# lxm0851/mp3

Hardware: AMD Instinct MI355X
Metric: stereo MP3 frames/s (128 kbps 44.1 kHz) at 1/2/4/8 GPU; % HBM roofline (higher is better)
Workload: dtype f32; 1 GPU; C3: full Layer III decode (Huffman->PCM), 65536 streams x 32 frames per GPU per step; streams_per_gpu=65536, hz=44100, seed=default, parallelism=streams sharded, 1 process per GPU, no data-path collective

## Files before the change

### abx/variants.py

```python
#!/usr/bin/env python3
import sys

import stage

KERNELS = ["mp3d_demux.hip", "mp3d_huffman.hip", "mp3d_synth.hip", "mp3d_demux_dev.h", "mp3d_huffman_dev.h", "mp3d_internal.h"]


def variant(name, reps):
    srcs = {k: open("mp3_amd/csrc/" + k).read() for k in KERNELS}
    flags = [b for a, b in reps if a == "FLAGS"]
    reps = [(a, b) for a, b in reps if a != "FLAGS"]
    for a, b in reps:
        assert any(a in s for s in srcs.values()), (name, a)
        srcs = {k: s.replace(a, b) for k, s in srcs.items()}
    stage.build("/tmp/vars/" + name, "build_ab/%s.so" % name, srcs, extra=flags)


W4H = ("__global__ void __launch_bounds__(HUFF_BLOCK) k_huffman(",
       "__global__ void __launch_bounds__(HUFF_BLOCK) __attribute__((amdgpu_waves_per_eu(4, 8))) k_huffman(")
_QS = "            /* ---------------- phase Q: requantise + stereo -> LDS ---------- */"
_IS = "            /* ---------------- phase I: alias + IMDCT + overlap ------------ */"
_MS = "            /* ---------------- phase M: matrixing on the matrix cores ------- */"
_WS = "            /* ---------------- phase W: 512-tap window -> PCM --------------- */"

# ... 713 lines not shown
                                   "+v"(xbp[6]), "+v"(xbp[7]));"""),
]

VARS["PHT"] = [
    ("    float *const sBuf = Wd.buf;\n",
     "    float *const sBuf = Wd.buf;\n    unsigned long long ph_[4] = {0ull, 0ull, 0ull, 0ull}, tQ_ = 0ull, tI_ = 0ull, tM_ = 0ull, tW_ = 0ull;\n"),
    (_QS, "            tQ_ = clock64();\n" + _QS),
    (_IS, "            tI_ = clock64(); ph_[0] += tI_ - tQ_;\n" + _IS),
    (_MS, "            tM_ = clock64(); ph_[1] += tM_ - tI_;\n" + _MS),
    (_WS, "            tW_ = clock64(); ph_[2] += tW_ - tM_;\n" + _WS),
    ("            wave_sync(); /* X reads done before the next granule's xr */",
     "            wave_sync(); /* X reads done before the next granule's xr */\n            ph_[3] += clock64() - tW_;"),
    ("    if (f1 == F && PF != 1) {",
     "    if ((blockIdx.x == 0 || blockIdx.x == 4000) && threadIdx.x == 0 && !SRC_XR && !LSF)\n"
     "        printf(\"PHT blk %d Q %llu I %llu M %llu W %llu\\n\", (int)blockIdx.x, ph_[0], ph_[1], ph_[2], ph_[3]);\n"
     "    if (f1 == F && PF != 1) {"),
]

VARS["PHT2"] = [
    ("    float *const sBuf = Wd.buf;\n",
     "    float *const sBuf = Wd.buf;\n    unsigned long long ph_[8] = {0ull, 0ull, 0ull, 0ull, 0ull, 0ull, 0ull, 0ull}, tQ_ = 0ull, tI_ = 0ull, tM_ = 0ull, tW_ = 0ull, tE_ = 0ull, t1_ = 0ull, t2_ = 0ull;\n"),
    (_QS, "            tQ_ = clock64(); if (tE_) ph_[7] += tQ_ - tE_;\n" + _QS),
    ("                (void)m12a;\n", "                (void)m12a;\n                t1_ = clock64(); ph_[4] += t1_ - tQ_;\n"),
    ("                xin();\n                } /* !fusedq */", "                t2_ = clock64(); ph_[5] += t2_ - t1_;\n                xin();\n                } /* !fusedq */"),
    (_IS, "            tI_ = clock64(); ph_[0] += tI_ - tQ_; ph_[6] += tI_ - t2_;\n" + _IS),
    (_MS, "            tM_ = clock64(); ph_[1] += tM_ - tI_;\n" + _MS),
    (_WS, "            tW_ = clock64(); ph_[2] += tW_ - tM_;\n" + _WS),
    ("            wave_sync(); /* X reads done before the next granule's xr */",
     "            wave_sync(); /* X reads done before the next granule's xr */\n            tE_ = clock64(); ph_[3] += tE_ - tW_;"),
    ("    if (f1 == F && PF != 1) {",
     "    if ((blockIdx.x == 0 || blockIdx.x == 4000) && threadIdx.x == 0 && !SRC_XR && !LSF)\n"
     "        printf(\"PHT2 blk %d Q %llu (Q1 %llu Q2 %llu Q3 %llu) I %llu M %llu W %llu G %llu\\n\", (int)blockIdx.x, ph_[0], ph_[4], ph_[5], ph_[6], ph_[1], ph_[2], ph_[3], ph_[7]);\n"
     "    if (f1 == F && PF != 1) {"),
]

VARS["PHT3"] = [
    ("    float *const sBuf = Wd.buf;\n",
     "    float *const sBuf = Wd.buf;\n    unsigned long long ph_[8] = {0ull, 0ull, 0ull, 0ull, 0ull, 0ull, 0ull, 0ull}, tQ_ = 0ull, t1_ = 0ull, ta_ = 0ull, tb_ = 0ull, tc_ = 0ull;\n"),
    ("                (void)m12a;\n", "                (void)m12a;\n                t1_ = clock64();\n"),
    ("                else read_cis(std::integral_constant<int, 5>{});\n",
     "                else read_cis(std::integral_constant<int, 5>{});\n                __asm__ volatile(\"s_waitcnt lgkmcnt(0)\" : \"+v\"(cis[0][0]), \"+v\"(cis[1][0]), \"+v\"(cis[0][1]), \"+v\"(cis[1][1]));\n                ta_ = clock64(); ph_[0] += ta_ - t1_;\n"),
    ("                else requant(std::integral_constant<int, 5>{});\n",
     "                else requant(std::integral_constant<int, 5>{});\n                __asm__ volatile(\"s_waitcnt lgkmcnt(0)\" : \"+v\"(xp[0][0]), \"+v\"(xp[1][0]));\n                tb_ = clock64(); ph_[1] += tb_ - ta_;\n"),
    ("                if (ms_fold) {\n",
     "                tc_ = clock64(); ph_[2] += tc_ - tb_;\n                if (ms_fold) {\n"),
    ("                xin();\n                } /* !fusedq */", "                ph_[3] += clock64() - tc_;\n                xin();\n                } /* !fusedq */"),
    ("    if (f1 == F && PF != 1) {",
     "    if ((blockIdx.x == 0 || blockIdx.x == 4000) && threadIdx.x == 0 && !SRC_XR && !LSF)\n"
     "        printf(\"PHT3 blk %d cis %llu requant %llu esc+stereo %llu scatter %llu\\n\", (int)blockIdx.x, ph_[0], ph_[1], ph_[2], ph_[3]);\n"
     "    if (f1 == F && PF != 1) {"),
]

VARS["MSZ"] = [
    ("""                            scatter(i, 0, xp[0][i] + xp[1][i]);
                            scatter(i, 1, xp[0][i] - xp[1][i]);""",
     """                            if (i < 2 || i < nlive) {
                                scatter(i, 0, xp[0][i] + xp[1][i]);
                                scatter(i, 1, xp[0][i] - xp[1][i]);
                            } else {
                                scatter(i, 0, (f32x2){0.f, 0.f});
                                scatter(i, 1, (f32x2){0.f, 0.f});
                            }"""),
]

VARS["MH"] = [
    ("    for (int f = fw; f < f1; f++) {\n        int nch, sr, mode = 0, mext = 0;",
     "    const int mlane_ = (int)(threadIdx.x & 63);\n"
     "    const uint32_t m_off_a = (uint32_t)(((mlane_ & 15) * SROW + 4 * (mlane_ >> 4)) * 4);\n"
     "    const uint32_t m_off_c = (uint32_t)((((mlane_ & 15) < 4 ? 32 + (mlane_ & 15) : 35) * SROW + 4 * (mlane_ >> 4)) * 4);\n"
# ... 329 lines not shown
```

### mp3_amd/csrc/mp3d_batch.cpp

```cpp
#include "mp3d_host.h"

using namespace mp3d;

hipError_t mp3d::state_clear(StreamState *st, int n, hipStream_t s) {
    hipError_t e = hipMemsetAsync(st, 0, sizeof(StreamState) * (size_t)n, s);
    if (e == hipSuccess)
        e = hipMemset2DAsync(&st[0].fmt, sizeof(StreamState), MP3D_STATE_FMT_BYTE, sizeof(uint32_t), (size_t)n, s);
    return e;
}

static bool poison_env() {
    const char *e = getenv("MP3D_DEBUG_POISON");
    return e && e[0] && strcmp(e, "0") != 0;
}

static int seg_frames(int n, int F, int n_cu, int min_len) {
    int seg_len = F;
    const long long want = 4LL * 4 * n_cu;
    if ((long long)n < want && F >= 2 * min_len) {
        const int nseg = (int)std::min<long long>((want + n - 1) / n, F / min_len);
        seg_len = (F + nseg - 1) / nseg;
    }
    const char *e = getenv("MP3D_SEG_FRAMES");
    if (e && atoi(e) > 0) seg_len = std::min(F, atoi(e));
// ... 167 lines not shown
    return MP3D_OK;
}

extern "C" int mp3d_batch_kernel_times(mp3d_batch *b, float *us3) {
    if (!b || !us3) return MP3D_E_ARG;
    if (!b->timing) return MP3D_E_ARG;
    HIPCHK(hipEventSynchronize(b->ev[3]));
    for (int i = 0; i < 3; i++) {
        float ms = 0;
        HIPCHK(hipEventElapsedTime(&ms, b->ev[i], b->ev[i + 1]));
        us3[i] = ms * 1000.f;
    }
    return MP3D_OK;
}

#define MP3D_WIDE_STREAMS 256
static bool demux_wide(int n) {
    const char *e = getenv("MP3D_DEMUX");
    if (e && !strcmp(e, "lane")) return true;
    if (e && !strcmp(e, "wave")) return false;
    return n >= MP3D_WIDE_STREAMS;
}

#define MP3D_WAVE_HUFF_UNITS 1024
static bool huffman_wave(int n_units) {
    const char *e = getenv("MP3D_HUFF");
    if (e && !strcmp(e, "wave")) return true;
    if (e && !strcmp(e, "lane")) return false;
    return n_units <= MP3D_WAVE_HUFF_UNITS;
}

#define MP3D_GEO_CACHE_STREAMS (1 << 30)

int mp3d::prepare_geometry(mp3d_batch *b, const uint64_t *offsets, const uint32_t *sizes, int n, hipStream_t s) {
    {
        mp3d_batch::Geo &g = b->geo[b->geo_i];
        if (n <= MP3D_GEO_CACHE_STREAMS && g.n == n && !memcmp(g.h, offsets, sizeof(uint64_t) * n) &&
            !memcmp(g.h + 2 * (size_t)n, sizes, sizeof(uint32_t) * n)) {
            HIPCHK(hipStreamWaitEvent(s, g.staged, 0));
            return MP3D_OK;
        }
    }
    b->geo_i ^= 1;
    mp3d_batch::Geo &g = b->geo[b->geo_i];
    g.n = -1;
    HIPCHK(hipEventSynchronize(g.staged));
// ... 87 lines not shown
    const bool inf_host = infos && !mapped && !is_device_ptr(infos, b->device);
    mp3d_frame_info *dinf = infos && !inf_host ? infos : b->d_infos.p;
    int r = fp ? run_front_fp(b, *fp, F, s, dinf) : run_front(b, frames, offsets, sizes, n, F, s, &sync_needed, mapped, dinf);
    if (r) return r;
    if (async && !mapped) return MP3D_E_ARG;
    const size_t PB = f32 ? sizeof(float) : sizeof(int16_t), row = 2304 * PB;
    const size_t pcm_bytes = (size_t)n * F * row;
    void *dpcm = pcm;
    const PtrKind pk = mapped ? PTR_DEV : ptr_kind(pcm, b->device);
    bool pcm_host = pk == PTR_HOST;
    if (pk != PTR_DEV) {
        r = b->d_pcm.grow(b, pcm_bytes);
        if (r) return r;
        dpcm = b->d_pcm;
        if (pk == PTR_OTHER_DEV) HIPCHK(hipMemcpyAsync(dpcm, pcm, pcm_bytes, hipMemcpyDefault, s));
    }
    DeviceCtx &dc = g_dev[b->device];
    const int seg_len = seg_len_req > 0 ? std::min(F, seg_len_req) : seg_frames(n, F, dc.n_cu, 4);
    TailPlan tp;
    r = tail_plan(b, n, F, seg_len, s, &tp);
    if (r) return r;
    if (b->poison) launch_lds_poison(dc.n_cu, s);
    launch_synth(b->rec, b->is_buf, b->meta, dc.tables, b->st, dpcm, f32, n, F, kinds, seg_len, tp.out, tp.in,
                 b->fam_ok ? b->d_work + 1 : nullptr, b->call_seq, dc.n_cu, s);
    if (b->timing) HIPCHK(hipEventRecord(b->ev[3], s));
    HIPCHK(hipGetLastError());
    tail_commit(b, n, F, seg_len, tp);
    const size_t ib = sizeof(mp3d_frame_info) * (size_t)n * F;
    if (pcm_host && !overwrite) {
        std::vector<mp3d_frame_info> tmp;
        mp3d_frame_info *hi = inf_host ? infos : nullptr;
        if (!hi) {
            tmp.resize((size_t)n * F);
            hi = tmp.data();
        }
        HIPCHK(hipMemcpyAsync(hi, dinf, ib, hipMemcpyDefault, s));
        HIPCHK(hipStreamSynchronize(s));
        std::vector<size_t> at;
        std::vector<uint8_t> kept;
        for (size_t i = 0; i < (size_t)n * F; i++) {
            const size_t w = (size_t)hi[i].samples * (size_t)hi[i].channels * PB;
            if (w >= row) continue;
            at.push_back(i);
            kept.insert(kept.end(), (const uint8_t *)pcm + i * row + w, (const uint8_t *)pcm + (i + 1) * row);
        }
        HIPCHK(hipMemcpyAsync(pcm, dpcm, pcm_bytes, hipMemcpyDeviceToHost, s));
        HIPCHK(hipStreamSynchronize(s));
// ... 245 lines not shown
```

### mp3_amd/csrc/mp3d_launch.h

```cpp
#ifndef MP3D_LAUNCH_H
#define MP3D_LAUNCH_H

#include <hip/hip_runtime.h>
#include <stdint.h>

struct StreamState; struct FrameRec; struct UnitMeta; struct DevTables;
struct RsState; struct RsCfg; struct RsPlan; struct RsLong;
struct FtState; struct FtPlan; struct FtTab;
struct LdState; struct LdPlan; struct LdTab;
struct TpState; struct TpPlan;

namespace mp3d {

hipError_t upload_demux_constants(const uint16_t *frame_bytes);
void launch_demux(const uint8_t *in, const uint64_t *in_off, const uint32_t *in_len, uint8_t *md,
                  const uint64_t *md_off, StreamState *st, FrameRec *rec, uint64_t *sideu, void *infos, int n_streams,
                  int F, int opts, bool wide, uint32_t *fam, uint32_t seq, hipStream_t strm);
void launch_demux_fp(const uint8_t *in, uint32_t len, const uint32_t *fo, uint8_t *md, StreamState *st,
                     const float *tail_in, StreamState *snap, FrameRec *rec, uint64_t *sideu, void *infos, int F,
                     int opts, hipStream_t strm);

void launch_huffman(const uint8_t *md, const uint64_t *md_off, const FrameRec *rec, const uint64_t *sideu,
                    const DevTables *tab, int16_t *is_buf, UnitMeta *meta, int n_streams, int F, int n_cu, bool wave,
                    uint32_t *work, uint32_t *rank, hipStream_t strm);

hipError_t upload_synth_constants(const float *win36, const float *is_ratio, const float *pow2q, const float *is_lsf);
hipError_t upload_frame_constants(const uint16_t *frame_bytes);
void launch_frame(const uint8_t *in_host, uint32_t in_have, const uint64_t *in_off, const uint32_t *in_len,
                  uint8_t *md, const uint64_t *md_off, StreamState *st, FrameRec *rec, uint64_t *sideu, void *infos,
                  int opts, const DevTables *tab, int16_t *is_buf, UnitMeta *meta, void *pcm, bool f32, bool lsf,
                  uint32_t *done, uint32_t seq, hipStream_t strm);
void launch_synth(const FrameRec *rec, const int16_t *is_buf, const UnitMeta *meta, const DevTables *tab,
                  StreamState *st, void *pcm, bool f32, int n_streams, int F, int kinds, int seg_len, float *st_tail,
                  const float *st_tail_in, const uint32_t *fam, uint32_t seq, int n_cu, hipStream_t strm);
void launch_synth_xr(const float *xr, const uint8_t *bt, const uint8_t *mixed, const DevTables *tab, StreamState *st,
                     int16_t *pcm, int n_streams, int F, int nch, int sr, int seg_len, float *st_tail,
                     const float *st_tail_in, hipStream_t strm);
void launch_lds_poison(int n_cu, hipStream_t strm);
void launch_gather_frames(const void *src, void *dst, const void *isrc, void *idst, const int *a, int L, int F, int k0,
                          int n_out, int bytes_per_row, hipStream_t strm);
#ifdef MP3D_WG_LDS_POISON
int wglds_probe_words();
void launch_wglds_probe(int n_cu, int n_groups, uint32_t *out, hipStream_t strm);
#endif

void launch_resample(const float *rows, const void *infos, RsState *st, const StreamState *sst, const RsCfg *cfg,
                     int out_ch, const float *tab, RsPlan *plan, int32_t *prefix, void *out, bool f32,
                     int32_t *out_count, int n, int F, long long stride, int tiles, int flush, int gapless,
                     hipStream_t strm);
void launch_resample_long(const float *rows, const void *infos, const int *a, const uint32_t *tag, const RsCfg *cfg,
                          int out_ch, const float *tab, RsLong *st, int32_t *prefix, void *out, bool f32, long long cap,
                          int L, int F, int k0, int n_out, int tiles, int first, int last, int gapless, hipStream_t strm);

void launch_features(const float *samples, const int32_t *counts, FtState *st, FtPlan *plan, const FtTab *tab, float *feat,
                     int32_t *feat_count, int n, long long sample_stride, long long feat_stride, int tiles, int flush,
                     hipStream_t strm);

// ... 19 lines not shown
```

### mp3_amd/csrc/mp3d_synth.hip

```cpp
#include "mp3d_device.h"
#include "mp3d_consts.h"
#define MP3D_DEMUX_TU frame_tu
#include "mp3d_demux_dev.h"
#include "mp3d_huffman_dev.h"
#include "mp3d_launch.h"

namespace mp3d {

__constant__ float c_win36[4][36];
__constant__ float c_is_ratio[7][2];
__constant__ float c_pow2q[4];
__constant__ float c_is_lsf[2][16][2];

__device__ __forceinline__ void dct3_9(const float *a, float *v) {
    const float C10 = 9.848077530e-01f;
    const float C20 = 9.396926208e-01f;
    const float C30 = 8.660254038e-01f;
    const float C40 = 7.660444431e-01f;
    const float C50 = 6.427876097e-01f;
    const float C70 = 3.420201433e-01f;
    const float C80 = 1.736481777e-01f;
    const float ev0 = fmaf(a[8], C80, fmaf(a[6], 0.5f, fmaf(a[4], C40, fmaf(a[2], C20, a[0]))));
    const float od0 = fmaf(a[7], C70, fmaf(a[5], C50, fmaf(a[3], C30, a[1] * C10)));
    v[0] = ev0 + od0;
// ... 163 lines not shown
    for (int i = tid; i < 32 * 16; i += NT)
        ((float *)&T.dwp[0][0])[((i & 15) >> 1) * 64 + (i >> 4) * 2 + (i & 1)] = (&tab->dwin[0][0])[i] * (F32 ? 1.0f : 32768.0f);
    if (tid < 7 + 9) {
        const float c9[7] = DCT9_KC, k9[9] = IMDCT36_K;
        T.kc[tid] = tid < 7 ? (f32x2){c9[tid], c9[tid]} : (f32x2){k9[tid - 7], -k9[tid - 7]};
    }
    if (tid < 4) T.p2q[tid] = pow2_quarter(tid);
    if (tid < 128) {
        const int l = tid & 63, c = l >> 5, j = l & 31;
        const int w = (tid >> 6) ? tab->win_b[j] : tab->win_a[j];
        T.xcol[tid >> 6][l] = (uint16_t)(18 * c * XROW + (w & 1) * 16 + (w >> 1));
    }
    for (int k = tid; k < 2 * 4 * 9; k += NT) {
        const int par = k / 36, bt = (k / 9) % 4, i = k % 9;
        const float *w = c_win36[bt];
        const float sa = (par && (i & 1)) ? -1.f : 1.f, sb = (par && !(i & 1)) ? -1.f : 1.f;
        T.wp[par][bt][i] = (f32x4){sa * w[i], sb * w[17 - i], sa * w[18 + i], sb * w[35 - i]};
    }
    if (LSF) {
        if (tid < 64) (&T.isr[0][0])[tid] = (&c_is_lsf[0][0][0])[tid];
    } else if (tid < 14) (&T.isr[0][0])[tid] = (&c_is_ratio[0][0])[tid];
}

template <bool SRC_XR, bool F32, bool LSF, int PF = 0>
__device__ __forceinline__ void synth_stream(const FrameRec *__restrict__ rec, const int16_t *__restrict__ is_buf,
                                             const UnitMeta *__restrict__ meta, const float *__restrict__ xr_in,
                                             const uint8_t *__restrict__ xr_bt, const uint8_t *__restrict__ xr_mixed,
                                             const DevTables *__restrict__ tab, StreamState *__restrict__ st,
                                             void *__restrict__ pcm, int F, int xr_nch, int xr_sr, int seg_len,
                                             float *__restrict__ st_tail, const float *__restrict__ st_tail_in,
                                             SynShared<LSF> &T, SynWave &Wd, int s, int seg, int nseg,
                                             float *xch = nullptr, uint32_t *isq = nullptr) {
    static_assert(PF == 0 || (!SRC_XR && !LSF), "PF: k_frame's MPEG-1 decode path only");
    const int f0 = seg * seg_len, f1 = min(F, f0 + seg_len);
    int fw = seg ? f0 - 1 : 0;
    int wlast = -1;
    bool from_state = seg == 0, ch1_state = false;
    if (!SRC_XR && seg > 0) {
        const uint32_t *rw = (const uint32_t *)(rec + (size_t)s * F);
        auto audio = [&](int f) {
            const uint32_t r4 = __builtin_amdgcn_readfirstlane(rw[8 * f + 4]);
            const uint32_t r6 = __builtin_amdgcn_readfirstlane(rw[8 * f + 6]);
            return (r4 & 0xFFFFu) != 0u && !(((r6 >> 8) & 0xFFu) & (REC_TAG | REC_DROP));
        };
        auto stereo = [&](int f) { return (__builtin_amdgcn_readfirstlane(rw[8 * f + 5]) >> 24) == 2u; };
        const int need = LSF ? 2 : 1;
        int found = 0, fa = f0;
// ... 218 lines not shown
            const uint32_t r5 = (uint32_t)__builtin_amdgcn_readlane((int)wr[0], 37);
            const uint32_t r6 = (uint32_t)__builtin_amdgcn_readlane((int)wr[0], 38);
            const uint32_t first_gr = (r6 >> 8) & 0xFFu;
            if (!(r4 & 0xFFFFu) || (first_gr & (REC_TAG | REC_DROP))) {
                if (f + 1 < f1) prefetch_full(2 * (f + 1));
                WAIT_VMCNT0();
                continue;
            }
            nch = (int)(r5 >> 24);
            sr = (int)((r6 >> 16) & 15u) - (LSF ? 3 : 0);
            mode = (int)(r5 >> 22) & 3;
            mext = (int)(r5 >> 20) & 3;
        }
        const uint64_t amask = nch == 2 ? ~0ull : 0xFFFFFFFFull;
        const uint32_t(*lpair)[288] = T.lpair[sr];
#pragma unroll
        for (int gr = PF == 2 ? 1 : 0; gr < (LSF || PF == 1 ? 1 : 2); gr++) {
            const int cs = PAR ? gr : 0;
            const int lane = opaque((int)(threadIdx.x & 63));
            const int ch = lane >> 5, sb = lane & 31;
            int bt0, mx0, bt1 = 0, mx1 = 0;
            if (!SRC_XR) __builtin_amdgcn_s_setprio(1);
            bool fusedq = false;
            float xf[18], up[8], dn[8];
            auto xin = [&]() {
                wave_sync();
                typedef __attribute__((address_space(3))) const f32x2 lds_cf2;
                lds_cf2 *const P = (lds_cf2 *)(uintptr_t)((uint32_t)(uintptr_t)(lds_cf32 *)(const float *)sBuf + xin_off);
#pragma unroll
                for (int i = 0; i < 9; i++) {
                    const f32x2 v = P[4 + i];
                    xf[2 * i] = v.x;
                    xf[2 * i + 1] = v.y;
                }
#pragma unroll
                for (int i = 0; i < 4; i++) {
                    const f32x2 p = P[i];
                    const f32x2 n = P[13 + i];
                    up[7 - 2 * i] = p.x;
                    up[6 - 2 * i] = p.y;
                    dn[2 * i] = n.x;
                    dn[2 * i + 1] = n.y;
                }
            };
            if (SRC_XR) {
                (void)fr;
                f32x2 cx[2][5];
#pragma unroll
                for (int c = 0; c < 2; c++)
#pragma unroll
                    for (int i = 0; i < 5; i++)
// ... 8 lines not shown
                    bt1 = __builtin_amdgcn_readlane((int)nbt, 1);
                    mx1 = bt1 == 2 ? __builtin_amdgcn_readlane((int)nbt, 3) : 0;
                }
                if (f + 1 < f1 || gr == 0) load_xr(2 * f + gr + 1);
                const int xv[2] = {bt0 == 2 ? (mx0 ? 2 : 1) : 0, bt1 == 2 ? (mx1 ? 2 : 1) : 0};
#pragma unroll
                for (int i = 0; i < 5; i++) {
                    if (i < 4 || lane < 32) {
                        const int k = lane + 64 * i;
#pragma unroll
                        for (int c = 0; c < 2; c++) {
                            if (c < nch) {
                                if (xv[c] == 0) {
                                    *(f32x2 *)&sBuf[576 * c + 2 * k] = cx[c][i];
                                } else {
                                    const uint32_t tv2 = lpair[xv[c]][k];
                                    sBuf[576 * c + ((tv2 >> 8) & 1023u)] = cx[c][i][0];
                                    sBuf[576 * c + ((tv2 >> 18) & 1023u)] = cx[c][i][1];
                                }
                            }
                        }
                    }
                }
                xin();
            } else {
                const int nzq0 = __builtin_amdgcn_readlane((int)wm[cs], 12) & 0xFFFF;
                const int nzq1 = nch == 2 ? __builtin_amdgcn_readlane((int)wm[cs], MW + 12) & 0xFFFF : 0;
                const int nzmax = nzq0 > nzq1 ? nzq0 : nzq1;
                const int nlive = nzmax <= 256 ? 2 : (nzmax <= 384 ? 3 : 5);
                uint32_t cis[2][5];
                auto read_cis = [&](auto nic) {
                    constexpr int NI = decltype(nic)::value;
#pragma unroll
                    for (int c = 0; c < 2; c++)
#pragma unroll
                        for (int i = 0; i < 5; i++)
                            cis[c][i] = i < NI ? (PAR ? isq[320 * c + 64 * i + lane] : nis[c][i]) : 0u;
                };
                if (lane < nch * MW) ((uint32_t *)&Wd.m[0])[lane] = wm[cs];
                const uint32_t m10a = (uint32_t)__builtin_amdgcn_readlane((int)wm[cs], 10);
                const uint32_t m11a = (uint32_t)__builtin_amdgcn_readlane((int)wm[cs], 11);
                const uint32_t m12a = (uint32_t)__builtin_amdgcn_readlane((int)wm[cs], 12);
                const uint32_t m10b = (uint32_t)__builtin_amdgcn_readlane((int)wm[cs], MW + 10);
                const uint32_t m11b = (uint32_t)__builtin_amdgcn_readlane((int)wm[cs], MW + 11);
                const uint32_t m12b = (uint32_t)__builtin_amdgcn_readlane((int)wm[cs], MW + 12);
                bt0 = (int)(m10a >> 8) & 0xFF;
                mx0 = (int)(m10a >> 16) & 0xFF;
                if (nch == 2) {
                    bt1 = (int)(m10b >> 8) & 0xFF;
                    mx1 = (int)(m10b >> 16) & 0xFF;
                }
                const int var[2] = {bt0 == 2 ? (mx0 ? 2 : 1) : 0, bt1 == 2 ? (mx1 ? 2 : 1) : 0};
                const bool is_on = mode == 1 && nch == 2 && (mext & 1);
                const bool ms_fold = mode == 1 && nch == 2 && mext == 2;
                fusedq = PAR && var[0] == 0 && var[1] == 0 && !is_on && !ms_fold;
                const float rsq2 = 0.70710678118654752f;
                const float msf = __int_as_float(__builtin_amdgcn_readfirstlane(ms_fold ? 0x3f3504f3 : 0x3f800000));
                auto p2q = [&](int q) { return ldexpf(T.p2q[q & 3], q >> 2) * msf; };
                if (var[0] == 0 && (nch == 1 || var[1] == 0)) {
                    const int c = lane >> 5, bl = lane & 31, j = bl < 22 ? bl : 21;
                    const uint32_t g10 = c ? m10b : m10a, g11 = c ? m11b : m11a;
                    const int gain = (int)(g10 & 0xFFu) - 210, shift = (int)(g10 >> 24) + 1;
                    const uint32_t wd = (uint32_t)__shfl((int)wm[cs], c * MW + (j >> 2));
                    const int sf = (int)(wd >> (8 * (j & 3))) & 0xFF;
                    const int pre = (g11 & 0xFFu) ? (int)(MP3D_PRETAB_BITS >> (2 * j)) & 3 : 0;
                    const float v = p2q(gain - ((sf + pre) << shift));
                    if (bl < 22) Wd.scale[c][bl] = v;
                } else {
                    const bool lng = lane < 22;
                    const int b = (lane - 22) / 3, w = lane - 22 - 3 * b;
                    auto band_scale = [&](uint32_t g10, uint32_t g11, int cbase) {
                        const int gain = (int)(g10 & 0xFFu) - 210, shift = (int)(g10 >> 24) + 1;
                        const bool mixed = ((g10 >> 16) & 0xFFu) != 0u, preflag = (g11 & 0xFFu) != 0u;
                        int j = mixed ? 8 + 3 * (b - 3) + w : 3 * b + w;
                        j = lng ? lane : (j < 0 ? 0 : (j > 39 ? 39 : j));
                        const uint32_t wd = (uint32_t)__shfl((int)wm[cs], cbase + (j >> 2));
                        const int sf = (int)(wd >> (8 * (j & 3))) & 0xFF;
                        const int pre = preflag ? (int)(MP3D_PRETAB_BITS >> (2 * (lane & 31))) & 3 : 0;
// ... 31 lines not shown
                        xf[2 * m] = *(const float *)(p43b + (t & 0x7FCu)) * sc;
                        xf[2 * m + 1] = *(const float *)(p43b + ((t >> 16) & 0x7FCu)) * sc;
                    }
                    if (__ballot((bigf & 0xF800F800u) != 0u)) {
#pragma unroll
                        for (int m = 0; m < 9; m++) {
                            const uint32_t w = iw[m];
#pragma unroll
                            for (int e = 0; e < 2; e++) {
                                const int v = (int)(int16_t)(e ? (w >> 16) : (w & 0xFFFFu));
                                const int a = v < 0 ? -v : v;
                                if ((uint32_t)(v + 256) >= 512u) {
                                    const float mag = pow43_big(a) * *(lds_cf32 *)(uintptr_t)(scb | (lpw[m] & 0xFCu));
                                    xf[2 * m + e] = v < 0 ? -mag : mag;
                                }
                            }
                        }
                    }
#pragma unroll
                    for (int k = 0; k < 8; k++) {
                        up[k] = __int_as_float(__builtin_amdgcn_update_dpp(0, __float_as_int(xf[17 - k]), 0x138, 0xF, 0xF, false));
                        dn[k] = __int_as_float(__builtin_amdgcn_update_dpp(0, __float_as_int(xf[k]), 0x130, 0xF, 0xF, false));
                    }
                } else {
                if (nlive == 2) read_cis(std::integral_constant<int, 2>{});
                else if (nlive == 3) read_cis(std::integral_constant<int, 3>{});
                else read_cis(std::integral_constant<int, 5>{});
                auto requant = [&](auto nic) {
                constexpr int NI = decltype(nic)::value;
#pragma unroll
                for (int i = 0; i < 5; i++) {
                    const bool ok = i < 4 || lane < 32;
#pragma unroll
                    for (int c = 0; c < 2; c++) {
                        if (i >= NI) {
                            XV(c, 2 * i) = 0.f;
                            XV(c, 2 * i + 1) = 0.f;
                            continue;
                        }
                        const uint32_t tv2 = ok ? lpair[var[c]][lane + 64 * i] : 0u;
                        uint32_t t;
                        __asm__("v_pk_mad_u16 %0, %1, 4, %2 op_sel_hi:[1,0,0]" : "=v"(t) : "v"(cis[c][i]), "s"(k1024));
                        bigacc |= t;
                        const float sc = *(lds_cf32 *)(uintptr_t)(sc_base[c] | (tv2 & 0xFCu));
                        XV(c, 2 * i) = *(const float *)(p43b + (t & 0x7FCu)) * sc;
                        XV(c, 2 * i + 1) = *(const float *)(p43b + ((t >> 16) & 0x7FCu)) * sc;
// ... 79 lines not shown
                        *(f32x2 *)&sBuf[576 * c + 2 * lane + 128 * i] = v;
                    } else {
                        const uint32_t tv2 = lpair[var[c]][lane + 64 * i];
                        sBuf[576 * c + ((tv2 >> 8) & 1023u)] = v.x;
                        sBuf[576 * c + ((tv2 >> 18) & 1023u)] = v.y;
                    }
                };
                if (ms_fold) {
#pragma unroll
                    for (int i = 0; i < 5; i++)
                        if (i < 4 || lane < 32) {
                            scatter(i, 0, xp[0][i] + xp[1][i]);
                            scatter(i, 1, xp[0][i] - xp[1][i]);
                        }
                } else {
#pragma unroll
                    for (int i = 0; i < 5; i++)
                        if (i < 4 || lane < 32) {
#pragma unroll
                            for (int c = 0; c < 2; c++)
                                if (c < nch) scatter(i, c, xp[c][i]);
                        }
                }
                xin();
                }
                if (PF == 0 && (LSF ? f + 1 < f1 : (gr == 0 || f + 1 < f1))) prefetch(LSF ? 2 * f + 2 : 2 * f + gr + 1, cs);
            }
            wave_sync();
#undef XV
            if (!SRC_XR) __builtin_amdgcn_s_setprio(0);
            if (PF == 2) {
                __syncthreads();
#pragma unroll
                for (int i = 0; i < 9; i++) ovp[i] = (f32x2){xch[2 * i * 64 + lane], xch[(2 * i + 1) * 64 + lane]};
            }
            const int bt = ch ? bt1 : bt0, mixed = ch ? mx1 : mx0;
            float o18[18];
            f32x2 nvp[9];
            {
                const int base = ch * 576 + 18 * sb;
                float(&x)[18] = xf;
                (void)base;
                const bool upper = (bt != 2 && sb >= 1) || (bt == 2 && mixed && sb == 1);
                const bool lower = (bt != 2 && sb <= 30) || (bt == 2 && mixed && sb == 0);
#pragma unroll
                for (int k = 0; k < 8; k++) {
                    const float lo = x[17 - k], hi = x[k];
                    const float nh = fmaf(up[k], MP3D_K_ALIAS_CA[k], hi * MP3D_K_ALIAS_CS[k]);
                    const float nl = fmaf(-dn[k], MP3D_K_ALIAS_CA[k], lo * MP3D_K_ALIAS_CS[k]);
                    x[k] = upper ? nh : hi;
                    x[17 - k] = lower ? nl : lo;
                }
                const bool long_imdct = bt != 2 || (mixed && sb < 2);
                if (long_imdct) {
                    const f32x4 *wq = T.wp[sb & 1][bt == 2 ? 0 : bt];
                    f32x2 W[9];
                    imdct36_wp(x, W, (const f32x2 *)(uintptr_t)(uint32_t)opaque((int)(uintptr_t)(lds_cf32 *)(const float *)&T.kc[0]));
#pragma unroll
                    for (int i = 0; i < 9; i++) {
                        const f32x4 q = wq[i];
                        const f32x2 o = pfma(bc(W[8 - i].y), (f32x2){q.x, q.y}, ovp[i]);
                        o18[i] = o.x;
                        o18[17 - i] = o.y;
                        nvp[i] = bc(W[8 - i].x) * (f32x2){q.z, q.w};
                    }
                } else {
                    const float sgo = (sb & 1) ? -1.f : 1.f;
                    const f32x2 sgp[2] = {(f32x2){1.f, sgo}, (f32x2){sgo, 1.f}};
                    float z[24];
#pragma unroll
                    for (int i = 0; i < 24; i++) z[i] = 0.f;
#pragma unroll
                    for (int w = 0; w < 3; w++) {
                        float h[6];
// ... 236 lines not shown
        const f32x2 sgp[2] = {(f32x2){1.f, sgo}, (f32x2){sgo, 1.f}};
        float *ovo = st_tail ? st_tail + (size_t)s * TAIL : &S.overlap[0][0][0];
        float *ffo = ovo + sizeof(S.overlap) / 4;
#pragma unroll
        for (int i = 0; i < 9; i++) {
            const f32x2 t = ovp[i] * sgp[i & 1];
            ovo[(ch * 32 + sb) * 18 + i] = t.x;
            ovo[(ch * 32 + sb) * 18 + 17 - i] = t.y;
        }
        const float hsc = F32 ? 1.0f : 1.0f / 32768.0f;
#pragma unroll
        for (int tp = 0; tp < 8; tp++) {
            ffo[(ch * MP3D_FIFO_SLOTS + 2 * tp) * 32 + sb] = hp[tp].x * hsc;
            if (2 * tp + 1 < MP3D_FIFO_SLOTS) ffo[(ch * MP3D_FIFO_SLOTS + 2 * tp + 1) * 32 + sb] = hp[tp].y * hsc;
        }
    }
}

template <bool SRC_XR, bool LSF> struct SynCfg {
    static constexpr bool DMA = !LSF;
    static constexpr int WAVES = DMA ? 8 : 4;
};

template <bool SRC_XR, bool F32, bool LSF>
__global__ void __launch_bounds__((64 * SynCfg<SRC_XR, LSF>::WAVES))
    __attribute__((amdgpu_waves_per_eu(SynCfg<SRC_XR, LSF>::DMA ? 4 : 3, 8)))
k_synth(const FrameRec *__restrict__ rec, const int16_t *__restrict__ is_buf, const UnitMeta *__restrict__ meta,
        const float *__restrict__ xr_in, const uint8_t *__restrict__ xr_bt, const uint8_t *__restrict__ xr_mixed,
        const DevTables *__restrict__ tab, StreamState *__restrict__ st, void *__restrict__ pcm, int n_streams,
        int F, int xr_nch, int xr_sr, int seg_len, float *__restrict__ st_tail,
        const float *__restrict__ st_tail_in, const uint32_t *__restrict__ fam, uint32_t seq) {
    constexpr int SYN_WAVES = SynCfg<SRC_XR, LSF>::WAVES;
    struct Lds {
        float pad_[64];
        SynWave Wv[SYN_WAVES];
        SynShared<LSF> T;
        uint32_t isq[SynCfg<SRC_XR, LSF>::DMA ? SYN_WAVES : 1][2 * 320];
    };
    static_assert(offsetof(Lds, T) + sizeof(SynShared<LSF>) <= 65536, "k_synth: tables within DS offset reach");
    static_assert(LSF || SRC_XR || sizeof(Lds) <= 160 * 1024 / 2, "k_synth: LDS for two workgroups per CU");
    __shared__ __attribute__((aligned(16))) Lds L;
    MP3D_LDS_ENTRY();
    SynShared<LSF> &T = L.T;
    SynWave *Wv = L.Wv;
    auto &s_isq = L.isq;
    if (LSF && !SRC_XR && fam && *fam != seq) return;
    if (!SRC_XR && !(LSF && fam)) {
        bool any = false;
        const int nsg = (F + seg_len - 1) / seg_len;
#pragma unroll
        for (int k = 0; k < SYN_WAVES; k++) {
            const int sk = (blockIdx.x * SYN_WAVES + k) / nsg;
            if (sk < n_streams) any |= (st[sk].kind == 2) == LSF;
        }
        if (!any) return;
    }
    synth_tables<F32, LSF, 64 * SYN_WAVES>(T, tab, threadIdx.x);
    __syncthreads();
    const int wid = __builtin_amdgcn_readfirstlane((int)(threadIdx.x >> 6));
    const int nseg = (F + seg_len - 1) / seg_len;
    const int nblk = (n_streams * nseg + SYN_WAVES - 1) / SYN_WAVES;
    auto run = [&](int blk) {
        const int vs = blk * SYN_WAVES + wid;
        if (vs >= n_streams * nseg) return false;
        const int s = vs / nseg, seg = vs - s * nseg;
        if (!SRC_XR && (st[s].kind == 2) != LSF) return true;
        synth_stream<SRC_XR, F32, LSF>(rec, is_buf, meta, xr_in, xr_bt, xr_mixed, tab, st, pcm, F, xr_nch, xr_sr,
                                       seg_len, st_tail, st_tail_in, T, Wv[wid], s, seg, nseg, nullptr,
                                       SynCfg<SRC_XR, LSF>::DMA ? s_isq[SynCfg<SRC_XR, LSF>::DMA ? wid : 0] : nullptr);
        return true;
    };
    if constexpr (LSF && !SRC_XR) {
        for (int blk = blockIdx.x; blk < nblk; blk += gridDim.x)
            if (!run(blk)) break;
    } else {
        run(blockIdx.x);
    }
}
__global__ void __launch_bounds__(256) k_gather_frames(const uint4 *__restrict__ src, uint4 *__restrict__ dst,
                                                       const DevInfo *__restrict__ isrc, DevInfo *__restrict__ idst,
                                                       const int *__restrict__ a, int L, int F, int k0, int row16) {
    MP3D_LDS_ENTRY();
    const int jl = blockIdx.x;
    const int k = jl / L;
    const int j = (k0 + k) * L + jl % L;
    const size_t sf = (size_t)k * F + (j - a[k]);
    const DevInfo inf = isrc[sf];
    const int lim = inf.samples * inf.channels * row16 / 2304;
    for (int i = threadIdx.x; i < row16; i += blockDim.x)
        dst[(size_t)jl * row16 + i] = i < lim ? src[sf * row16 + i] : make_uint4(0u, 0u, 0u, 0u);
    if (idst && threadIdx.x == 0) idst[jl] = isrc[sf];
}
// ... 95 lines not shown
}

hipError_t upload_frame_constants(const uint16_t *frame_bytes) { return upload_demux_tables(frame_bytes); }

void launch_frame(const uint8_t *in_host, uint32_t in_have, const uint64_t *in_off, const uint32_t *in_len,
                  uint8_t *md, const uint64_t *md_off, StreamState *st, FrameRec *rec, uint64_t *sideu, void *infos,
                  int opts, const DevTables *tab, int16_t *is_buf, UnitMeta *meta, void *pcm, bool f32, bool lsf,
                  uint32_t *done, uint32_t seq, hipStream_t strm) {
#define MP3D_FRAME_LAUNCH(F32_, LSF_)                                                                              \
    hipLaunchKernelGGL((k_frame<F32_, LSF_>), dim3(1), dim3(256), 0, strm, in_host, in_have, in_off, in_len, md,    \
                       md_off, st, rec, sideu, (DevInfo *)infos, opts, tab, is_buf, meta, pcm, done, seq)
    if (f32) {
        if (lsf) MP3D_FRAME_LAUNCH(true, true);
        else MP3D_FRAME_LAUNCH(true, false);
    } else {
        if (lsf) MP3D_FRAME_LAUNCH(false, true);
        else MP3D_FRAME_LAUNCH(false, false);
    }
#undef MP3D_FRAME_LAUNCH
}

void launch_synth(const FrameRec *rec, const int16_t *is_buf, const UnitMeta *meta, const DevTables *tab,
                  StreamState *st, void *pcm, bool f32, int n_streams, int F, int kinds, int seg_len, float *st_tail,
                  const float *st_tail_in, const uint32_t *fam, uint32_t seq, int n_cu, hipStream_t strm) {
    const int waves = n_streams * ((F + seg_len - 1) / seg_len);
    const int lsf_grid = 3 * (n_cu > 0 ? n_cu : 256);
#define MP3D_SYNTH_LAUNCH(F32_, LSF_)                                                                              \
    do {                                                                                                           \
        constexpr int NW = SynCfg<false, LSF_>::WAVES;                                                             \
        int nb = (waves + NW - 1) / NW;                                                                            \
        if (LSF_ && fam && nb > lsf_grid) nb = lsf_grid;                                                           \
        hipLaunchKernelGGL((k_synth<false, F32_, LSF_>), dim3(nb), dim3(64 * NW), 0, strm, rec, is_buf, meta,       \
                           (const float *)nullptr, (const uint8_t *)nullptr, (const uint8_t *)nullptr, tab, st, pcm,  \
                           n_streams, F, 2, 0, seg_len, st_tail, st_tail_in, LSF_ ? fam : nullptr, seq);           \
    } while (0)
    if (f32) {
        if (kinds & 1) MP3D_SYNTH_LAUNCH(true, false);
        if (kinds & 2) MP3D_SYNTH_LAUNCH(true, true);
    } else {
        if (kinds & 1) MP3D_SYNTH_LAUNCH(false, false);
        if (kinds & 2) MP3D_SYNTH_LAUNCH(false, true);
    }
#undef MP3D_SYNTH_LAUNCH
}

void launch_synth_xr(const float *xr, const uint8_t *bt, const uint8_t *mixed, const DevTables *tab, StreamState *st,
                     int16_t *pcm, int n_streams, int F, int nch, int sr, int seg_len, float *st_tail,
                     const float *st_tail_in, hipStream_t strm) {
    const int waves = n_streams * ((F + seg_len - 1) / seg_len);
    constexpr int NW = SynCfg<true, false>::WAVES;
    hipLaunchKernelGGL((k_synth<true, false, false>), dim3((waves + NW - 1) / NW), dim3(64 * NW), 0,
                       strm, (const FrameRec *)nullptr, (const int16_t *)nullptr, (const UnitMeta *)nullptr, xr, bt,
                       mixed, tab, st, (void *)pcm, n_streams, F, nch, sr, seg_len, st_tail, st_tail_in,
                       (const uint32_t *)nullptr, 0u);
}

#define LDS_POISON_WORDS (160 * 1024 / 4)
__device__ __forceinline__ void lds_fill_all(uint32_t *s, uint32_t word) {
    volatile uint32_t *v = s;
    for (int i = threadIdx.x; i < LDS_POISON_WORDS; i += 1024) v[i] = word;
}

__global__ void __launch_bounds__(1024) k_lds_poison() {
    __shared__ uint32_t s[LDS_POISON_WORDS];
// ... 53 lines not shown
```

Baseline: 203.2 million frames/s.

## Add specialised long-block MS-stereo requant path and masked alias butterflies in synth

Adds a LONGQ template variant of the synth kernel, on by default through an env switch. It gives granules that are all long blocks with MS stereo a specialised requantise path, which reads coefficients, applies pow43 and scale, folds M/S and writes straight to LDS. Only the live chunks are processed, and the xin window offset is redirected to a zeroed chunk. Alias butterflies now use exec-masked inline asm with literal constants instead of per-element selects. The cost is an extra kernel instantiation, raw asm exec manipulation and more code size or register pressure.

Measured after the change: 207.2 million frames/s, median of 6. +2.0%, better.

```diff
diff --git a/abx/variants.py b/abx/variants.py
--- a/abx/variants.py
+++ b/abx/variants.py
@@ -759,7 +759,7 @@
      "    float *const sBuf = Wd.buf;\n    unsigned long long ph_[8] = {0ull, 0ull, 0ull, 0ull, 0ull, 0ull, 0ull, 0ull}, tQ_ = 0ull, tI_ = 0ull, tM_ = 0ull, tW_ = 0ull, tE_ = 0ull, t1_ = 0ull, t2_ = 0ull;\n"),
     (_QS, "            tQ_ = clock64(); if (tE_) ph_[7] += tQ_ - tE_;\n" + _QS),
     ("                (void)m12a;\n", "                (void)m12a;\n                t1_ = clock64(); ph_[4] += t1_ - tQ_;\n"),
-    ("                xin();\n                } /* !fusedq */", "                t2_ = clock64(); ph_[5] += t2_ - t1_;\n                xin();\n                } /* !fusedq */"),
+    ("                xin(xin_off);\n                } /* !fusedq */", "                t2_ = clock64(); ph_[5] += t2_ - t1_;\n                xin(xin_off);\n                } /* !fusedq */"),
     (_IS, "            tI_ = clock64(); ph_[0] += tI_ - tQ_; ph_[6] += tI_ - t2_;\n" + _IS),
     (_MS, "            tM_ = clock64(); ph_[1] += tM_ - tI_;\n" + _MS),
     (_WS, "            tW_ = clock64(); ph_[2] += tW_ - tM_;\n" + _WS),
@@ -781,7 +781,7 @@
      "                else requant(std::integral_constant<int, 5>{});\n                __asm__ volatile(\"s_waitcnt lgkmcnt(0)\" : \"+v\"(xp[0][0]), \"+v\"(xp[1][0]));\n                tb_ = clock64(); ph_[1] += tb_ - ta_;\n"),
     ("                if (ms_fold) {\n",
      "                tc_ = clock64(); ph_[2] += tc_ - tb_;\n                if (ms_fold) {\n"),
-    ("                xin();\n                } /* !fusedq */", "                ph_[3] += clock64() - tc_;\n                xin();\n                } /* !fusedq */"),
+    ("                xin(xin_off);\n                } /* !fusedq */", "                ph_[3] += clock64() - tc_;\n                xin(xin_off);\n                } /* !fusedq */"),
     ("    if (f1 == F && PF != 1) {",
      "    if ((blockIdx.x == 0 || blockIdx.x == 4000) && threadIdx.x == 0 && !SRC_XR && !LSF)\n"
      "        printf(\"PHT3 blk %d cis %llu requant %llu esc+stereo %llu scatter %llu\\n\", (int)blockIdx.x, ph_[0], ph_[1], ph_[2], ph_[3]);\n"
diff --git a/mp3_amd/csrc/mp3d_batch.cpp b/mp3_amd/csrc/mp3d_batch.cpp
--- a/mp3_amd/csrc/mp3d_batch.cpp
+++ b/mp3_amd/csrc/mp3d_batch.cpp
@@ -213,6 +213,11 @@
     return n >= MP3D_WIDE_STREAMS;
 }
 
+static bool synth_longpath() {
+    const char *e = getenv("MP3D_SYNTH_LONGPATH");
+    return !(e && !strcmp(e, "0"));
+}
+
 #define MP3D_WAVE_HUFF_UNITS 1024
 static bool huffman_wave(int n_units) {
     const char *e = getenv("MP3D_HUFF");
@@ -346,7 +351,7 @@
     if (r) return r;
     if (b->poison) launch_lds_poison(dc.n_cu, s);
     launch_synth(b->rec, b->is_buf, b->meta, dc.tables, b->st, dpcm, f32, n, F, kinds, seg_len, tp.out, tp.in,
-                 b->fam_ok ? b->d_work + 1 : nullptr, b->call_seq, dc.n_cu, s);
+                 b->fam_ok ? b->d_work + 1 : nullptr, b->call_seq, dc.n_cu, synth_longpath(), s);
     if (b->timing) HIPCHK(hipEventRecord(b->ev[3], s));
     HIPCHK(hipGetLastError());
     tail_commit(b, n, F, seg_len, tp);
diff --git a/mp3_amd/csrc/mp3d_launch.h b/mp3_amd/csrc/mp3d_launch.h
--- a/mp3_amd/csrc/mp3d_launch.h
+++ b/mp3_amd/csrc/mp3d_launch.h
@@ -32,7 +32,8 @@
                   uint32_t *done, uint32_t seq, hipStream_t strm);
 void launch_synth(const FrameRec *rec, const int16_t *is_buf, const UnitMeta *meta, const DevTables *tab,
                   StreamState *st, void *pcm, bool f32, int n_streams, int F, int kinds, int seg_len, float *st_tail,
-                  const float *st_tail_in, const uint32_t *fam, uint32_t seq, int n_cu, hipStream_t strm);
+                  const float *st_tail_in, const uint32_t *fam, uint32_t seq, int n_cu, bool longpath,
+                  hipStream_t strm);
 void launch_synth_xr(const float *xr, const uint8_t *bt, const uint8_t *mixed, const DevTables *tab, StreamState *st,
                      int16_t *pcm, int n_streams, int F, int nch, int sr, int seg_len, float *st_tail,
                      const float *st_tail_in, hipStream_t strm);
diff --git a/mp3_amd/csrc/mp3d_synth.hip b/mp3_amd/csrc/mp3d_synth.hip
--- a/mp3_amd/csrc/mp3d_synth.hip
+++ b/mp3_amd/csrc/mp3d_synth.hip
@@ -209,7 +209,7 @@
     } else if (tid < 14) (&T.isr[0][0])[tid] = (&c_is_ratio[0][0])[tid];
 }
 
-template <bool SRC_XR, bool F32, bool LSF, int PF = 0>
+template <bool SRC_XR, bool F32, bool LSF, int PF = 0, bool LONGQ = false>
 __device__ __forceinline__ void synth_stream(const FrameRec *__restrict__ rec, const int16_t *__restrict__ is_buf,
                                              const UnitMeta *__restrict__ meta, const float *__restrict__ xr_in,
                                              const uint8_t *__restrict__ xr_bt, const uint8_t *__restrict__ xr_mixed,
@@ -474,11 +474,14 @@
             int bt0, mx0, bt1 = 0, mx1 = 0;
             if (!SRC_XR) __builtin_amdgcn_s_setprio(1);
             bool fusedq = false;
+            auto all_long = [&]() {
+                return PAR && LONGQ && nch == 2 && mode == 1 && mext == 2 && bt0 != 2 && bt1 != 2;
+            };
             float xf[18], up[8], dn[8];
-            auto xin = [&]() {
+            auto xin = [&](uint32_t xoff) {
                 wave_sync();
                 typedef __attribute__((address_space(3))) const f32x2 lds_cf2;
-                lds_cf2 *const P = (lds_cf2 *)(uintptr_t)((uint32_t)(uintptr_t)(lds_cf32 *)(const float *)sBuf + xin_off);
+                lds_cf2 *const P = (lds_cf2 *)(uintptr_t)((uint32_t)(uintptr_t)(lds_cf32 *)(const float *)sBuf + xoff);
 #pragma unroll
                 for (int i = 0; i < 9; i++) {
                     const f32x2 v = P[4 + i];
@@ -533,7 +536,7 @@
                         }
                     }
                 }
-                xin();
+                xin(xin_off);
             } else {
                 const int nzq0 = __builtin_amdgcn_readlane((int)wm[cs], 12) & 0xFFFF;
                 const int nzq1 = nch == 2 ? __builtin_amdgcn_readlane((int)wm[cs], MW + 12) & 0xFFFF : 0;
@@ -565,6 +568,7 @@
                 const bool is_on = mode == 1 && nch == 2 && (mext & 1);
                 const bool ms_fold = mode == 1 && nch == 2 && mext == 2;
                 fusedq = PAR && var[0] == 0 && var[1] == 0 && !is_on && !ms_fold;
+                const bool longq = all_long();
                 const float rsq2 = 0.70710678118654752f;
                 const float msf = __int_as_float(__builtin_amdgcn_readfirstlane(ms_fold ? 0x3f3504f3 : 0x3f800000));
                 auto p2q = [&](int q) { return ldexpf(T.p2q[q & 3], q >> 2) * msf; };
@@ -642,6 +646,72 @@
                         up[k] = __int_as_float(__builtin_amdgcn_update_dpp(0, __float_as_int(xf[17 - k]), 0x138, 0xF, 0xF, false));
                         dn[k] = __int_as_float(__builtin_amdgcn_update_dpp(0, __float_as_int(xf[k]), 0x130, 0xF, 0xF, false));
                     }
+                } else if (longq) {
+                    auto qlong = [&](auto nic) {
+                        constexpr int NI = decltype(nic)::value;
+                        uint32_t w[2][NI];
+#pragma unroll
+                        for (int c = 0; c < 2; c++)
+#pragma unroll
+                            for (int i = 0; i < NI; i++) w[c][i] = isq[320 * c + 64 * i + lane];
+                        f32x2 x[2][NI];
+                        uint32_t big = 0u;
+#pragma unroll
+                        for (int i = 0; i < NI; i++) {
+                            const uint32_t tv2 = (i < 4 || lane < 32) ? lpair[0][lane + 64 * i] : 0u;
+#pragma unroll
+                            for (int c = 0; c < 2; c++) {
+                                uint32_t t;
+                                __asm__("v_pk_mad_u16 %0, %1, 4, %2 op_sel_hi:[1,0,0]" : "=v"(t) : "v"(w[c][i]), "s"(k1024));
+                                big |= t;
+                                const float sc = *(lds_cf32 *)(uintptr_t)(sc_base[c] | (tv2 & 0xFCu));
+                                x[c][i] = (f32x2){*(const float *)(p43b + (t & 0x7FCu)) * sc,
+                                                  *(const float *)(p43b + ((t >> 16) & 0x7FCu)) * sc};
+                            }
+                        }
+                        if (__ballot((big & 0xF800F800u) != 0u)) {
+#pragma unroll
+                            for (int i = 0; i < NI; i++) {
+#pragma unroll
+                                for (int c = 0; c < 2; c++) {
+#pragma unroll
+                                    for (int e = 0; e < 2; e++) {
+                                        const int v = (int)(int16_t)(e ? (w[c][i] >> 16) : (w[c][i] & 0xFFFFu));
+                                        const int a = v < 0 ? -v : v;
+                                        if ((uint32_t)(v + 256) >= 512u) {
+                                            const uint32_t tv2 = lpair[0][lane + 64 * i];
+                                            const float mag = pow43_big(a) * Wd.scale[c][(tv2 >> 2) & 63u];
+                                            x[c][i][e] = v < 0 ? -mag : mag;
+                                        }
+                                    }
+                                }
+                            }
+                        }
+#pragma unroll
+                        for (int i = 0; i < NI; i++)
+                            if (i < 4 || lane < 32) {
+                                *(f32x2 *)&sBuf[2 * lane + 128 * i] = x[0][i] + x[1][i];
+                                *(f32x2 *)&sBuf[576 + 2 * lane + 128 * i] = x[0][i] - x[1][i];
+                            }
+                        if constexpr (NI < 5) {
+                            f32x2 z0;
+                            __asm__ volatile("v_mov_b64 %0, 0" : "=v"(z0));
+                            if (NI < 4 || lane < 32) {
+                                *(f32x2 *)&sBuf[2 * lane + 128 * NI] = z0;
+                                *(f32x2 *)&sBuf[576 + 2 * lane + 128 * NI] = z0;
+                            }
+                            constexpr int SBD = (128 * NI + 8 + 17) / 18;
+                            static_assert(18 * SBD - 8 >= 128 * NI && 18 * (SBD - 1) + 26 <= 128 * NI + (NI < 4 ? 128 : 64),
+                                          "k_synth: the zero chunk covers the windows that reach it");
+                            xin((lane & 31) >= SBD ? (uint32_t)(128 * NI * 4) : xin_off);
+                        } else {
+                            xin(xin_off);
+                        }
+                    };
+                    if (nzmax <= 256) qlong(std::integral_constant<int, 2>{});
+                    else if (nzmax <= 384) qlong(std::integral_constant<int, 3>{});
+                    else if (nzmax <= 512) qlong(std::integral_constant<int, 4>{});
+                    else qlong(std::integral_constant<int, 5>{});
                 } else {
                 if (nlive == 2) read_cis(std::integral_constant<int, 2>{});
                 else if (nlive == 3) read_cis(std::integral_constant<int, 3>{});
@@ -767,7 +837,7 @@
                                 if (c < nch) scatter(i, c, xp[c][i]);
                         }
                 }
-                xin();
+                xin(xin_off);
                 }
                 if (PF == 0 && (LSF ? f + 1 < f1 : (gr == 0 || f + 1 < f1))) prefetch(LSF ? 2 * f + 2 : 2 * f + gr + 1, cs);
             }
@@ -788,6 +858,69 @@
                 (void)base;
                 const bool upper = (bt != 2 && sb >= 1) || (bt == 2 && mixed && sb == 1);
                 const bool lower = (bt != 2 && sb <= 30) || (bt == 2 && mixed && sb == 0);
+                if (PAR && LONGQ) {
+                    const uint32_t mu0 = bt0 != 2 ? 0xFFFFFFFEu : (mx0 ? 2u : 0u), mu1 = bt1 != 2 ? 0xFFFFFFFEu : (mx1 ? 2u : 0u);
+                    const uint32_t ml0 = mu0 >> 1, ml1 = mu1 >> 1;
+                    auto m64 = [](uint32_t lo, uint32_t hi) {
+                        return (uint64_t)(uint32_t)__builtin_amdgcn_readfirstlane((int)lo) |
+                               ((uint64_t)(uint32_t)__builtin_amdgcn_readfirstlane((int)hi) << 32);
+                    };
+                    const uint64_t mup = m64(mu0, mu1), mlo = m64(ml0, ml1);
+#define ALIAS_BITS(A, k, v) static_assert(__builtin_bit_cast(uint32_t, A[k]) == v, "alias literal " #A)
+                    ALIAS_BITS(MP3D_K_ALIAS_CS, 0, 0x3f5b84a8u); ALIAS_BITS(MP3D_K_ALIAS_CS, 1, 0x3f61b9d8u);
+                    ALIAS_BITS(MP3D_K_ALIAS_CS, 2, 0x3f731addu); ALIAS_BITS(MP3D_K_ALIAS_CS, 3, 0x3f7bba81u);
+                    ALIAS_BITS(MP3D_K_ALIAS_CS, 4, 0x3f7eda41u); ALIAS_BITS(MP3D_K_ALIAS_CS, 5, 0x3f7fc8fdu);
+                    ALIAS_BITS(MP3D_K_ALIAS_CS, 6, 0x3f7ff965u); ALIAS_BITS(MP3D_K_ALIAS_CS, 7, 0x3f7fff8du);
+                    ALIAS_BITS(MP3D_K_ALIAS_CA, 0, 0xbf03b5feu); ALIAS_BITS(MP3D_K_ALIAS_CA, 1, 0xbef186dau);
+                    ALIAS_BITS(MP3D_K_ALIAS_CA, 2, 0xbea07302u); ALIAS_BITS(MP3D_K_ALIAS_CA, 3, 0xbe3a4774u);
+                    ALIAS_BITS(MP3D_K_ALIAS_CA, 4, 0xbdc1b01du); ALIAS_BITS(MP3D_K_ALIAS_CA, 5, 0xbd27cb87u);
+                    ALIAS_BITS(MP3D_K_ALIAS_CA, 6, 0xbc68a11du); ALIAS_BITS(MP3D_K_ALIAS_CA, 7, 0xbb727b46u);
+#undef ALIAS_BITS
+                    __asm__ volatile("s_mov_b64 exec, %16\n\t"
+                                     "v_mul_f32 %0, 0x3f5b84a8, %0\n\t"
+                                     "v_mul_f32 %1, 0x3f61b9d8, %1\n\t"
+                                     "v_mul_f32 %2, 0x3f731add, %2\n\t"
+                                     "v_mul_f32 %3, 0x3f7bba81, %3\n\t"
+                                     "v_mul_f32 %4, 0x3f7eda41, %4\n\t"
+                                     "v_mul_f32 %5, 0x3f7fc8fd, %5\n\t"
+                                     "v_mul_f32 %6, 0x3f7ff965, %6\n\t"
+                                     "v_mul_f32 %7, 0x3f7fff8d, %7\n\t"
+                                     "v_fmac_f32 %0, 0xbf03b5fe, %8\n\t"
+                                     "v_fmac_f32 %1, 0xbef186da, %9\n\t"
+                                     "v_fmac_f32 %2, 0xbea07302, %10\n\t"
+                                     "v_fmac_f32 %3, 0xbe3a4774, %11\n\t"
+                                     "v_fmac_f32 %4, 0xbdc1b01d, %12\n\t"
+                                     "v_fmac_f32 %5, 0xbd27cb87, %13\n\t"
+                                     "v_fmac_f32 %6, 0xbc68a11d, %14\n\t"
+                                     "v_fmac_f32 %7, 0xbb727b46, %15\n\t"
+                                     "s_mov_b64 exec, -1"
+                                     : "+v"(x[0]), "+v"(x[1]), "+v"(x[2]), "+v"(x[3]), "+v"(x[4]), "+v"(x[5]),
+                                       "+v"(x[6]), "+v"(x[7])
+                                     : "v"(up[0]), "v"(up[1]), "v"(up[2]), "v"(up[3]), "v"(up[4]), "v"(up[5]), "v"(up[6]),
+                                       "v"(up[7]), "s"(mup));
+                    __asm__ volatile("s_mov_b64 exec, %16\n\t"
+                                     "v_mul_f32 %0, 0x3f5b84a8, %0\n\t"
+                                     "v_mul_f32 %1, 0x3f61b9d8, %1\n\t"
+                                     "v_mul_f32 %2, 0x3f731add, %2\n\t"
+                                     "v_mul_f32 %3, 0x3f7bba81, %3\n\t"
+                                     "v_mul_f32 %4, 0x3f7eda41, %4\n\t"
+                                     "v_mul_f32 %5, 0x3f7fc8fd, %5\n\t"
+                                     "v_mul_f32 %6, 0x3f7ff965, %6\n\t"
+                                     "v_mul_f32 %7, 0x3f7fff8d, %7\n\t"
+                                     "v_fmac_f32 %0, 0x3f03b5fe, %8\n\t"
+                                     "v_fmac_f32 %1, 0x3ef186da, %9\n\t"
+                                     "v_fmac_f32 %2, 0x3ea07302, %10\n\t"
+                                     "v_fmac_f32 %3, 0x3e3a4774, %11\n\t"
+                                     "v_fmac_f32 %4, 0x3dc1b01d, %12\n\t"
+                                     "v_fmac_f32 %5, 0x3d27cb87, %13\n\t"
+                                     "v_fmac_f32 %6, 0x3c68a11d, %14\n\t"
+                                     "v_fmac_f32 %7, 0x3b727b46, %15\n\t"
+                                     "s_mov_b64 exec, -1"
+                                     : "+v"(x[17]), "+v"(x[16]), "+v"(x[15]), "+v"(x[14]), "+v"(x[13]),
+                                       "+v"(x[12]), "+v"(x[11]), "+v"(x[10])
+                                     : "v"(dn[0]), "v"(dn[1]), "v"(dn[2]), "v"(dn[3]), "v"(dn[4]), "v"(dn[5]), "v"(dn[6]),
+                                       "v"(dn[7]), "s"(mlo));
+                } else {
 #pragma unroll
                 for (int k = 0; k < 8; k++) {
                     const float lo = x[17 - k], hi = x[k];
@@ -795,6 +928,7 @@
                     const float nl = fmaf(-dn[k], MP3D_K_ALIAS_CA[k], lo * MP3D_K_ALIAS_CS[k]);
                     x[k] = upper ? nh : hi;
                     x[17 - k] = lower ? nl : lo;
+                }
                 }
                 const bool long_imdct = bt != 2 || (mixed && sb < 2);
                 if (long_imdct) {
@@ -1077,7 +1211,7 @@
     static constexpr int WAVES = DMA ? 8 : 4;
 };
 
-template <bool SRC_XR, bool F32, bool LSF>
+template <bool SRC_XR, bool F32, bool LSF, bool LONGQ = false>
 __global__ void __launch_bounds__((64 * SynCfg<SRC_XR, LSF>::WAVES))
     __attribute__((amdgpu_waves_per_eu(SynCfg<SRC_XR, LSF>::DMA ? 4 : 3, 8)))
 k_synth(const FrameRec *__restrict__ rec, const int16_t *__restrict__ is_buf, const UnitMeta *__restrict__ meta,
@@ -1120,9 +1254,9 @@
         if (vs >= n_streams * nseg) return false;
         const int s = vs / nseg, seg = vs - s * nseg;
         if (!SRC_XR && (st[s].kind == 2) != LSF) return true;
-        synth_stream<SRC_XR, F32, LSF>(rec, is_buf, meta, xr_in, xr_bt, xr_mixed, tab, st, pcm, F, xr_nch, xr_sr,
-                                       seg_len, st_tail, st_tail_in, T, Wv[wid], s, seg, nseg, nullptr,
-                                       SynCfg<SRC_XR, LSF>::DMA ? s_isq[SynCfg<SRC_XR, LSF>::DMA ? wid : 0] : nullptr);
+        synth_stream<SRC_XR, F32, LSF, 0, LONGQ>(
+            rec, is_buf, meta, xr_in, xr_bt, xr_mixed, tab, st, pcm, F, xr_nch, xr_sr, seg_len, st_tail, st_tail_in, T,
+            Wv[wid], s, seg, nseg, nullptr, SynCfg<SRC_XR, LSF>::DMA ? s_isq[SynCfg<SRC_XR, LSF>::DMA ? wid : 0] : nullptr);
         return true;
     };
     if constexpr (LSF && !SRC_XR) {
@@ -1264,24 +1398,27 @@
 
 void launch_synth(const FrameRec *rec, const int16_t *is_buf, const UnitMeta *meta, const DevTables *tab,
                   StreamState *st, void *pcm, bool f32, int n_streams, int F, int kinds, int seg_len, float *st_tail,
-                  const float *st_tail_in, const uint32_t *fam, uint32_t seq, int n_cu, hipStream_t strm) {
+                  const float *st_tail_in, const uint32_t *fam, uint32_t seq, int n_cu, bool longpath,
+                  hipStream_t strm) {
     const int waves = n_streams * ((F + seg_len - 1) / seg_len);
     const int lsf_grid = 3 * (n_cu > 0 ? n_cu : 256);
-#define MP3D_SYNTH_LAUNCH(F32_, LSF_)                                                                              \
+#define MP3D_SYNTH_LAUNCH(F32_, LSF_, LONGQ_)                                                                      \
     do {                                                                                                           \
         constexpr int NW = SynCfg<false, LSF_>::WAVES;                                                             \
         int nb = (waves + NW - 1) / NW;                                                                            \
         if (LSF_ && fam && nb > lsf_grid) nb = lsf_grid;                                                           \
-        hipLaunchKernelGGL((k_synth<false, F32_, LSF_>), dim3(nb), dim3(64 * NW), 0, strm, rec, is_buf, meta,       \
-                           (const float *)nullptr, (const uint8_t *)nullptr, (const uint8_t *)nullptr, tab, st, pcm,  \
-                           n_streams, F, 2, 0, seg_len, st_tail, st_tail_in, LSF_ ? fam : nullptr, seq);           \
+        hipLaunchKernelGGL((k_synth<false, F32_, LSF_, LONGQ_>), dim3(nb), dim3(64 * NW), 0, strm, rec, is_buf,     \
+                           meta, (const float *)nullptr, (const uint8_t *)nullptr, (const uint8_t *)nullptr, tab,   \
+                           st, pcm, n_streams, F, 2, 0, seg_len, st_tail, st_tail_in, LSF_ ? fam : nullptr, seq);   \
     } while (0)
     if (f32) {
-        if (kinds & 1) MP3D_SYNTH_LAUNCH(true, false);
-        if (kinds & 2) MP3D_SYNTH_LAUNCH(true, true);
+        if ((kinds & 1) && longpath) MP3D_SYNTH_LAUNCH(true, false, true);
+        if ((kinds & 1) && !longpath) MP3D_SYNTH_LAUNCH(true, false, false);
+        if (kinds & 2) MP3D_SYNTH_LAUNCH(true, true, false);
     } else {
-        if (kinds & 1) MP3D_SYNTH_LAUNCH(false, false);
-        if (kinds & 2) MP3D_SYNTH_LAUNCH(false, true);
+        if ((kinds & 1) && longpath) MP3D_SYNTH_LAUNCH(false, false, true);
+        if ((kinds & 1) && !longpath) MP3D_SYNTH_LAUNCH(false, false, false);
+        if (kinds & 2) MP3D_SYNTH_LAUNCH(false, true, false);
     }
 #undef MP3D_SYNTH_LAUNCH
 }
```
